# alexkroman/tiny-audio

Measured on AMD Instinct MI355X. Metric: training audio-sec/sec on 10s@16kHz clips, higher is better.
Workload: dtype bf16

## Files before the change

### tiny_audio_amd/csrc/attention.hip

```cpp
#include <cstdlib>
#include <type_traits>
#include "common.h"
#include "../../include/ta355.h"

#define KV_TILE 64
#define CT_STRIDE 128
#define LOG2E 1.4426950408889634f
#define NEG_BIG (-1.0e30f)

#ifdef TA355_ATTN_STAMPS
__device__ unsigned long long g_attn_stamps[8192 * 16];
#define ATTN_STAMP(blk, i, who) do { if (threadIdx.x == (who)) g_attn_stamps[(long)(blk) * 16 + (i)] = __builtin_amdgcn_s_memtime(); } while (0)
extern "C" int ta_debug_attn_stamps(unsigned long long* host_out, int nblocks) {
  return hipMemcpyFromSymbol(host_out, HIP_SYMBOL(g_attn_stamps), (size_t)nblocks * 16 * sizeof(unsigned long long)) == hipSuccess ? 0 : 2;
}
#else
#define ATTN_STAMP(blk, i, who) do { } while (0)
#endif

template <int HD> struct RowTile {
  static constexpr int STRIDE = HD * 2;
  static constexpr int BYTES = 64 * STRIDE;
  static __device__ __forceinline__ int swz(int r) { return HD == 64 ? ((r >> 1) & 7) : (r & 15); }
  static __device__ __forceinline__ int off(int r, int c) { return r * STRIDE + ((c ^ swz(r)) << 4); }
// ... 372 lines not shown
#pragma unroll
          for (int r = 0; r < 4; ++r) {
            const int key = key0 + kt * 16 + g * 4 + r;
            const bool v = (key <= qrow) & (mkv[r] != 0);
            s[sub][kt][r] = v ? s[sub][kt][r] : -INFINITY;
          }
        }
      }
      float mloc = max3(s[sub][0][0], s[sub][0][1], s[sub][0][2]);
      mloc = max3(mloc, s[sub][0][3], s[sub][1][0]);
      mloc = max3(mloc, s[sub][1][1], s[sub][1][2]);
      mloc = max3(mloc, s[sub][1][3], s[sub][2][0]);
      mloc = max3(mloc, s[sub][2][1], s[sub][2][2]);
      mloc = max3(mloc, s[sub][2][3], s[sub][3][0]);
      mloc = max3(mloc, s[sub][3][1], s[sub][3][2]);
      mloc = fmaxf(mloc, s[sub][3][3]);
      const float m_new = fmaxf(m_run[sub], group_max(mloc));
      if (__any(m_new != m_run[sub])) {
        const float alpha = __builtin_amdgcn_exp2f((m_run[sub] - m_new) * sl2);
#pragma unroll
        for (int i = 0; i <= ND; ++i) { o[sub][i][0] *= alpha; o[sub][i][1] *= alpha; o[sub][i][2] *= alpha; o[sub][i][3] *= alpha; }
        m_run[sub] = m_new;
      }
      const float mb = m_new * sl2;
#pragma unroll
      for (int kt = 0; kt < 4; ++kt)
#pragma unroll
        for (int r = 0; r < 4; ++r) s[sub][kt][r] = __builtin_amdgcn_exp2f(fmaf(s[sub][kt][r], sl2, -mb));
    }
#pragma unroll
    for (int kp = 0; kp < 2; ++kp) {
      bf16x8 pb[QSUB];
#pragma unroll
      for (int sub = 0; sub < QSUB; ++sub) pb[sub] = pack_p(s[sub][2 * kp], s[sub][2 * kp + 1]);
#pragma unroll
      for (int dt = 0; dt <= ND; ++dt) {
        const bf16x8 va = read_colfrag(Vt, dt * 16 + l15, (2 * kp) * 16 + g * 4, (2 * kp + 1) * 16 + g * 4);
#pragma unroll
        for (int sub = 0; sub < QSUB; ++sub)
          o[sub][dt] = __builtin_amdgcn_mfma_f32_16x16x32_bf16(va, pb[sub], o[sub][dt], 0, 0, 0);
        if (dt & 1) __builtin_amdgcn_sched_barrier(0);
      }
    }
  }
#pragma unroll
  for (int sub = 0; sub < QSUB; ++sub) {
    const int qrow = q0 + sub * 16 + l15;
    const float l_run = __shfl(o[sub][ND][0], l15, 64);
    if (qrow < L) {
      const float inv = l_run > 0.f ? 1.0f / l_run : 0.f;
      bf16_t* orow = O + ((long)b * L + qrow) * ((long)Hq * HD) + (long)h * HD;
#pragma unroll
      for (int dt = 0; dt < ND; dt += 2) {
        const uint32_t x0 = pack2bf(o[sub][dt][0] * inv, o[sub][dt][1] * inv), x1 = pack2bf(o[sub][dt][2] * inv, o[sub][dt][3] * inv);
        const uint32_t y0 = pack2bf(o[sub][dt + 1][0] * inv, o[sub][dt + 1][1] * inv), y1 = pack2bf(o[sub][dt + 1][2] * inv, o[sub][dt + 1][3] * inv);
        const auto a = __builtin_amdgcn_permlane16_swap(x0, y0, false, false);
        const auto c = __builtin_amdgcn_permlane16_swap(x1, y1, false, false);
        *(uint4*)(orow + 16 * (dt + (g & 1)) + 8 * (g >> 1)) = make_uint4(a[0], c[0], a[1], c[1]);
      }
      if (LSE && g == 0) LSE[(long)(b * Hq + h) * L + qrow] = l_run > 0.f ? m_run[sub] * scale + __logf(l_run) : 1.0e30f;
    }
  }
  }
}

__device__ __forceinline__ void dma16_asm(const void* g, unsigned lds) {
  asm volatile("s_mov_b32 m0, %0\n\ts_nop 0\n\tglobal_load_lds_dwordx4 %1, off" ::"s"(lds), "v"(g) : "memory");
}
__device__ __forceinline__ void dma_rowtile128(const bf16_t* base, long row_stride, int row0, int nrows, unsigned lds_tile, int wave,
                                               int lane) {
#pragma unroll
  for (int i = 0; i < 4; ++i) {
    const int blk = wave + 4 * i, r = blk * 4 + (lane >> 4);
    int gr = row0 + r; if (gr > nrows - 1) gr = nrows - 1; if (gr < 0) gr = 0;
    const int c = (lane & 15) ^ RowTile<128>::swz_tr(r);
    dma16_asm(base + (long)gr * row_stride + c * 8, __builtin_amdgcn_readfirstlane(lds_tile + blk * 1024));
  }
}
__device__ __forceinline__ unsigned lds_addr_of(const char* p) {
  return __builtin_amdgcn_readfirstlane((unsigned)(unsigned long)(const __attribute__((address_space(3))) char*)p);
}
constexpr int BWD_BUF = 2 * 64 * 128 * 2 + 512;

template <int HD, int MAXT, int QSUB, int NW, bool PAIR = false, bool NORM = true, bool ROPE = true>
__global__ __launch_bounds__(NW * 64) void attn_fwd_gqa_qkv_kernel(const bf16_t* __restrict__ qkv0, const float* __restrict__ qn_w,
                                                               const float* __restrict__ kn_w, const float* __restrict__ cosT,
                                                               const float* __restrict__ sinT, const int* __restrict__ pos,
                                                               bf16_t* __restrict__ Qo, bf16_t* __restrict__ Ko, bf16_t* __restrict__ Vo,
                                                               float* __restrict__ rq, float* __restrict__ rk, bf16_t* __restrict__ O,
                                                               float* __restrict__ LSE, const int* __restrict__ kmask, int B, int Hq,
                                                               int Hkv, int L, float scale, float eps) {
  static_assert(HD == 128, "Qwen3 head_dim");
  extern __shared__ __attribute__((aligned(16))) char smem[];
  constexpr int ND = HD / 16, NT_ = NW * 64;
  char* Ks = smem;
  char* Vs = smem + MAXT * RowTile<HD>::BYTES;
  int* Ms = (int*)(Vs + MAXT * RowTile<HD>::BYTES);
  const int tid = threadIdx.x, lane = tid & 63, wave = tid >> 6, g = lane >> 4, l15 = lane & 15;
  const int b = blockIdx.x / Hkv, hk = blockIdx.x % Hkv;
  const int grp = Hq / Hkv, cph = PAIR ? (L + 15) / 16 : (L + 16 * QSUB - 1) / (16 * QSUB), nchunk = PAIR ? cph : grp * cph;
  const long ld = (long)(Hq + 2 * Hkv) * HD;
  const float sl2 = scale * LOG2E;
  const int ntiles = (L + KV_TILE - 1) / KV_TILE;
  constexpr int PER = (MAXT * 64 * (HD / 8) + NT_ - 1) / NT_;
  ATTN_STAMP(blockIdx.x + 6144, 0, 0);
  {
    const unsigned ldsK = lds_addr_of(Ks), ldsV = lds_addr_of(Vs);
    const bf16_t* kbase = qkv0 + (long)b * L * ld + (long)(Hq + hk) * HD;
    const bf16_t* vbase = kbase + (long)Hkv * HD;
    for (int blk = wave; blk < ntiles * 16; blk += NW) {
      const int t = blk >> 4, rb4 = (blk & 15) * 4, r = rb4 + (lane >> 4);
      int gr = t * KV_TILE + r; if (gr > L - 1) gr = L - 1;
      const int c = (lane & 15) ^ RowTile<HD>::swz(r), cv = (lane & 15) ^ RowTile<HD>::swz_tr(r);
      const unsigned off = __builtin_amdgcn_readfirstlane((unsigned)(t * RowTile<HD>::BYTES + rb4 * 256));
      dma16_asm(kbase + (long)gr * ld + c * 8, ldsK + off);
      dma16_asm(vbase + (long)gr * ld + cv * 8, ldsV + off);
    }
  }
  {
    const int c = tid & 15;
    float wk[8];
    if constexpr (NORM) {
      const float4 wa = *(const float4*)(kn_w + c * 8), wb = *(const float4*)(kn_w + c * 8 + 4);
      wk[0] = wa.x; wk[1] = wa.y; wk[2] = wa.z; wk[3] = wa.w; wk[4] = wb.x; wk[5] = wb.y; wk[6] = wb.z; wk[7] = wb.w;
    }
    float4 cc[2][4];
    auto rope_rows = [&](int i, float4* dst) {
      if constexpr (!ROPE) return;
      const int ch = tid + i * NT_, t = ch / (64 * (HD / 8)), w = ch % (64 * (HD / 8));
      const int krow = t * KV_TILE + w / (HD / 8), gr = krow > L - 1 ? L - 1 : krow;
      const int pp = pos ? pos[(long)b * L + gr] : gr;
      const float* cp = cosT + (long)pp * 64 + (c & 7) * 8;
      const float* sp = sinT + (long)pp * 64 + (c & 7) * 8;
      dst[0] = *(const float4*)cp; dst[1] = *(const float4*)(cp + 4); dst[2] = *(const float4*)sp; dst[3] = *(const float4*)(sp + 4);
    };
    rope_rows(0, cc[0]);
    for (int i = tid; i < ntiles * 64; i += NT_) Ms[i] = (i < L) ? (kmask ? kmask[(long)b * L + i] : 1) : 0;
    ATTN_STAMP(blockIdx.x + 6144, 1, 0);
    asm volatile("s_waitcnt vmcnt(0)" ::: "memory");
    __syncthreads();
    ATTN_STAMP(blockIdx.x + 6144, 2, 0);
#pragma unroll
    for (int i = 0; i < PER; ++i) {
      const int ch = tid + i * NT_, t = ch / (64 * (HD / 8)), w = ch % (64 * (HD / 8));
      if (i + 1 < PER) rope_rows(i + 1, cc[(i + 1) & 1]);
      if (t < ntiles) {
        const int r = w / (HD / 8);
        const int krow = t * KV_TILE + r, gr = krow > L - 1 ? L - 1 : krow;
        const long tok = (long)b * L + gr;
        char* kp = Ks + t * RowTile<HD>::BYTES + RowTile<HD>::off(r, c);
        const uint4 kin = *(const uint4*)kp;
        const uint4 vin = *(const uint4*)(Vs + t * RowTile<HD>::BYTES + RowTile<HD>::off_tr(r, c));
        const uint32_t u[4] = {kin.x, kin.y, kin.z, kin.w};
        uint4 kv = kin;
        float rr = 1.f;
        if constexpr (NORM || ROPE) {
          float x[8];
#pragma unroll
          for (int k = 0; k < 4; ++k) { x[2 * k] = bf2f((bf16_t)(u[k] & 0xffff)); x[2 * k + 1] = bf2f((bf16_t)(u[k] >> 16)); }
          if constexpr (NORM) {
            float ss = 0.f;
#pragma unroll
            for (int e = 0; e < 8; ++e) ss += x[e] * x[e];
            ss = row_sum16(ss);
            rr = rsqrtf(ss / (float)HD + eps);
          }
          const float4* q4 = cc[i & 1];
          float cs[8], sn[8];
          if constexpr (ROPE) {
            cs[0] = q4[0].x; cs[1] = q4[0].y; cs[2] = q4[0].z; cs[3] = q4[0].w; cs[4] = q4[1].x; cs[5] = q4[1].y; cs[6] = q4[1].z; cs[7] = q4[1].w;
            sn[0] = q4[2].x; sn[1] = q4[2].y; sn[2] = q4[2].z; sn[3] = q4[2].w; sn[4] = q4[3].x; sn[5] = q4[3].y; sn[6] = q4[3].z; sn[7] = q4[3].w;
          }
          float y[8];
#pragma unroll
          for (int e = 0; e < 8; ++e) {
            const float n = NORM ? x[e] * rr * wk[e] : x[e];
            if constexpr (ROPE) {
              const float np = row_xor8(n);
              y[e] = c < 8 ? n * cs[e] - np * sn[e] : n * cs[e] + np * sn[e];
            } else {
              y[e] = n;
            }
          }
          kv = make_uint4(pack2bf(y[0], y[1]), pack2bf(y[2], y[3]), pack2bf(y[4], y[5]), pack2bf(y[6], y[7]));
          *(uint4*)kp = kv;
        }
        if (krow < L) {
          *(uint4*)(Ko + ((long)(b * Hkv + hk) * L + krow) * HD + c * 8) = kv;
          if (Vo) *(uint4*)(Vo + ((long)(b * Hkv + hk) * L + krow) * HD + c * 8) = vin;
          if (NORM && c == 0) rk[tok * Hkv + hk] = rr;
        }
      }
    }
  }
  ATTN_STAMP(blockIdx.x + 6144, 3, 0);
  __syncthreads();
  ATTN_STAMP(blockIdx.x + 6144, 4, 0);
  const bf16x8 ones = (bf16x8){0x3f80, 0x3f80, 0x3f80, 0x3f80, 0x3f80, 0x3f80, 0x3f80, 0x3f80};
  const bf16x8 zeros = (bf16x8){0, 0, 0, 0, 0, 0, 0, 0};
  const bf16x8 one_row = l15 == 0 ? ones : zeros;
  for (int pass = 0; pass < 2; ++pass) {
  const int chunk = pass == 0 ? wave : nchunk - 1 - wave;
  if (chunk >= nchunk || (pass == 1 && chunk < NW)) continue;
  const int h0 = PAIR ? hk * grp : hk * grp + chunk / cph;
  const int q0 = PAIR ? chunk * 16 : (chunk % cph) * 16 * QSUB;
  constexpr int RSTEP = PAIR ? 0 : 16;
  bf16x8 qf[QSUB][HD / 32];
  float4 tc[2][2], ts[2][2];
#pragma unroll
  for (int sub = 0; sub < QSUB; ++sub) {
    const int h = PAIR ? h0 + sub : h0;
    const int qrow = q0 + sub * RSTEP + l15, qr = qrow > L - 1 ? L - 1 : qrow;
    const long tok = (long)b * L + qr;
    const bf16_t* src = qkv0 + tok * ld + (long)h * HD;
    uint4 raw[HD / 32];
#pragma unroll
    for (int ks = 0; ks < HD / 32; ++ks) raw[ks] = *(const uint4*)(src + ks * 32 + g * 8);
    if (ROPE && (!PAIR || sub == 0)) {
      const int p = pos ? pos[tok] : qr;
#pragma unroll
      for (int ks = 0; ks < 2; ++ks) {
        const int d0 = ks * 32 + g * 8;
        tc[ks][0] = *(const float4*)(cosT + (long)p * 64 + d0); tc[ks][1] = *(const float4*)(cosT + (long)p * 64 + d0 + 4);
        ts[ks][0] = *(const float4*)(sinT + (long)p * 64 + d0); ts[ks][1] = *(const float4*)(sinT + (long)p * 64 + d0 + 4);
      }
    }
    float x[HD / 32][8], ss = 0.f;
#pragma unroll
    for (int ks = 0; ks < HD / 32; ++ks) {
      const uint32_t u[4] = {raw[ks].x, raw[ks].y, raw[ks].z, raw[ks].w};
#pragma unroll
      for (int k = 0; k < 4; ++k) { x[ks][2 * k] = bf2f((bf16_t)(u[k] & 0xffff)); x[ks][2 * k + 1] = bf2f((bf16_t)(u[k] >> 16)); }
      if constexpr (NORM) {
#pragma unroll
        for (int e = 0; e < 8; ++e) ss += x[ks][e] * x[ks][e];
      }
    }
    float rr = 1.f;
    if constexpr (NORM) { ss = group_sum(ss); rr = rsqrtf(ss / (float)HD + eps); }
#pragma unroll
    for (int ks = 0; ks < 2; ++ks) {
      const int d0 = ks * 32 + g * 8;
      float cs[8], sn[8], w1[8], w2[8];
      if constexpr (ROPE) {
        const float4 c0 = tc[ks][0], c1 = tc[ks][1], s0 = ts[ks][0], s1 = ts[ks][1];
        cs[0] = c0.x; cs[1] = c0.y; cs[2] = c0.z; cs[3] = c0.w; cs[4] = c1.x; cs[5] = c1.y; cs[6] = c1.z; cs[7] = c1.w;
        sn[0] = s0.x; sn[1] = s0.y; sn[2] = s0.z; sn[3] = s0.w; sn[4] = s1.x; sn[5] = s1.y; sn[6] = s1.z; sn[7] = s1.w;
      }
      if constexpr (NORM) {
        const float4 wa = *(const float4*)(qn_w + d0), wb = *(const float4*)(qn_w + d0 + 4);
        const float4 wc = *(const float4*)(qn_w + 64 + d0), wd = *(const float4*)(qn_w + 64 + d0 + 4);
        w1[0] = wa.x; w1[1] = wa.y; w1[2] = wa.z; w1[3] = wa.w; w1[4] = wb.x; w1[5] = wb.y; w1[6] = wb.z; w1[7] = wb.w;
        w2[0] = wc.x; w2[1] = wc.y; w2[2] = wc.z; w2[3] = wc.w; w2[4] = wd.x; w2[5] = wd.y; w2[6] = wd.z; w2[7] = wd.w;
      }
      float y1[8], y2[8];
#pragma unroll
      for (int e = 0; e < 8; ++e) {
        const float n1 = NORM ? x[ks][e] * rr * w1[e] : x[ks][e], n2 = NORM ? x[ks + 2][e] * rr * w2[e] : x[ks + 2][e];
        y1[e] = ROPE ? n1 * cs[e] - n2 * sn[e] : n1;
        y2[e] = ROPE ? n2 * cs[e] + n1 * sn[e] : n2;
      }
      union { bf16x8 v; uint4 u; } a, c;
      a.u = make_uint4(pack2bf(y1[0], y1[1]), pack2bf(y1[2], y1[3]), pack2bf(y1[4], y1[5]), pack2bf(y1[6], y1[7]));
      c.u = make_uint4(pack2bf(y2[0], y2[1]), pack2bf(y2[2], y2[3]), pack2bf(y2[4], y2[5]), pack2bf(y2[6], y2[7]));
      qf[sub][ks] = a.v; qf[sub][ks + 2] = c.v;
      if (qrow < L) {
        bf16_t* qdst = Qo + ((long)(b * Hq + h) * L + qrow) * HD;
        *(uint4*)(qdst + d0) = a.u;
        *(uint4*)(qdst + 64 + d0) = c.u;
      }
    }
    if (NORM && qrow < L && g == 0) rq[tok * Hq + h] = rr;
  }
  f32x4 o[QSUB][ND + 1];
#pragma unroll
  for (int sub = 0; sub < QSUB; ++sub)
#pragma unroll
    for (int i = 0; i <= ND; ++i) o[sub][i] = (f32x4){0.f, 0.f, 0.f, 0.f};
  float m_run[QSUB];
#pragma unroll
  for (int sub = 0; sub < QSUB; ++sub) m_run[sub] = NEG_BIG;
  const int my_tiles = min(ntiles, (q0 + (PAIR ? 16 : 16 * QSUB) - 1) / KV_TILE + 1);
  ATTN_STAMP(blockIdx.x + 6144, 5 + 3 * pass, 0);
  for (int t = 0; t < my_tiles; ++t) {
    const int key0 = t * KV_TILE;
    const char* Kt = Ks + t * RowTile<HD>::BYTES;
    const char* Vt = Vs + t * RowTile<HD>::BYTES;
    f32x4 s[QSUB][4];
#pragma unroll
    for (int kt = 0; kt < 4; ++kt) {
#pragma unroll
      for (int sub = 0; sub < QSUB; ++sub) s[sub][kt] = (f32x4){0.f, 0.f, 0.f, 0.f};
#pragma unroll
      for (int ks = 0; ks < HD / 32; ++ks) {
        const bf16x8 a = *(const bf16x8*)(Kt + RowTile<HD>::off(kt * 16 + l15, ks * 4 + g));
#pragma unroll
        for (int sub = 0; sub < QSUB; ++sub)
          s[sub][kt] = __builtin_amdgcn_mfma_f32_16x16x32_bf16(a, qf[sub][ks], s[sub][kt], 0, 0, 0);
      }
      __builtin_amdgcn_sched_barrier(0);
    }
#pragma unroll
    for (int sub = 0; sub < QSUB; ++sub) {
      const int qrow = q0 + sub * RSTEP + l15;
      const bool full = (key0 + KV_TILE <= L) && (kmask == nullptr) && (key0 + KV_TILE - 1 <= q0 + sub * RSTEP);
      if (!full) {
#pragma unroll
        for (int kt = 0; kt < 4; ++kt) {
          const int4 mk = *(const int4*)(Ms + key0 + kt * 16 + g * 4);
          const int mkv[4] = {mk.x, mk.y, mk.z, mk.w};
#pragma unroll
          for (int r = 0; r < 4; ++r) {
            const int key = key0 + kt * 16 + g * 4 + r;
            const bool v = (key <= qrow) & (mkv[r] != 0);
            s[sub][kt][r] = v ? s[sub][kt][r] : -INFINITY;
          }
        }
      }
      float mloc = max3(s[sub][0][0], s[sub][0][1], s[sub][0][2]);
      mloc = max3(mloc, s[sub][0][3], s[sub][1][0]);
      mloc = max3(mloc, s[sub][1][1], s[sub][1][2]);
      mloc = max3(mloc, s[sub][1][3], s[sub][2][0]);
      mloc = max3(mloc, s[sub][2][1], s[sub][2][2]);
      mloc = max3(mloc, s[sub][2][3], s[sub][3][0]);
      mloc = max3(mloc, s[sub][3][1], s[sub][3][2]);
      mloc = fmaxf(mloc, s[sub][3][3]);
      const float m_new = fmaxf(m_run[sub], group_max(mloc));
      if (__any(m_new != m_run[sub])) {
        const float alpha = __builtin_amdgcn_exp2f((m_run[sub] - m_new) * sl2);
#pragma unroll
        for (int i = 0; i <= ND; ++i) { o[sub][i][0] *= alpha; o[sub][i][1] *= alpha; o[sub][i][2] *= alpha; o[sub][i][3] *= alpha; }
        m_run[sub] = m_new;
      }
      const float mb = m_new * sl2;
#pragma unroll
      for (int kt = 0; kt < 4; ++kt)
#pragma unroll
        for (int r = 0; r < 4; ++r) s[sub][kt][r] = __builtin_amdgcn_exp2f(fmaf(s[sub][kt][r], sl2, -mb));
    }
#pragma unroll
    for (int kp = 0; kp < 2; ++kp) {
      bf16x8 pb[QSUB];
#pragma unroll
      for (int sub = 0; sub < QSUB; ++sub) pb[sub] = pack_p(s[sub][2 * kp], s[sub][2 * kp + 1]);
#pragma unroll
      for (int dt = 0; dt <= ND; ++dt) {
        const bf16x8 va = dt < ND ? read_colfrag_tr<HD>(Vt, dt, l15, (2 * kp) * 16 + g * 4, (2 * kp + 1) * 16 + g * 4) : one_row;
#pragma unroll
        for (int sub = 0; sub < QSUB; ++sub)
          o[sub][dt] = __builtin_amdgcn_mfma_f32_16x16x32_bf16(va, pb[sub], o[sub][dt], 0, 0, 0);
        if (dt & 1) __builtin_amdgcn_sched_barrier(0);
      }
    }
  }
  ATTN_STAMP(blockIdx.x + 6144, 6 + 3 * pass, 0);
#pragma unroll
  for (int sub = 0; sub < QSUB; ++sub) {
    const int h = PAIR ? h0 + sub : h0;
    const int qrow = q0 + sub * RSTEP + l15;
    const float l_run = __shfl(o[sub][ND][0], l15, 64);
    if (qrow < L) {
      const float inv = l_run > 0.f ? 1.0f / l_run : 0.f;
      bf16_t* orow = O + ((long)b * L + qrow) * ((long)Hq * HD) + (long)h * HD;
#pragma unroll
      for (int dt = 0; dt < ND; dt += 2) {
        const uint32_t x0 = pack2bf(o[sub][dt][0] * inv, o[sub][dt][1] * inv), x1 = pack2bf(o[sub][dt][2] * inv, o[sub][dt][3] * inv);
        const uint32_t y0 = pack2bf(o[sub][dt + 1][0] * inv, o[sub][dt + 1][1] * inv), y1 = pack2bf(o[sub][dt + 1][2] * inv, o[sub][dt + 1][3] * inv);
        const auto a = __builtin_amdgcn_permlane16_swap(x0, y0, false, false);
        const auto c = __builtin_amdgcn_permlane16_swap(x1, y1, false, false);
        *(uint4*)(orow + 16 * (dt + (g & 1)) + 8 * (g >> 1)) = make_uint4(a[0], c[0], a[1], c[1]);
      }
      if (LSE && g == 0) LSE[(long)(b * Hq + h) * L + qrow] = l_run > 0.f ? m_run[sub] * scale + __logf(l_run) : 1.0e30f;
    }
  }
  ATTN_STAMP(blockIdx.x + 6144, 7 + 3 * pass, 0);
  }
#ifdef TA355_ATTN_STAMPS
  asm volatile("s_waitcnt vmcnt(0)" ::: "memory");
  ATTN_STAMP(blockIdx.x + 6144, 11, 0);
#endif
}

struct QkvPostBwd {
  const bf16_t* qkv0;
  const float *rq, *rk;
  const float *qn_w, *kn_w;
  const float *cosT, *sinT;
  const int* pos;
  bf16_t* dqkv;
};
constexpr int QP_PITCH = 128 * 4 + 16;
__device__ __forceinline__ float oct_sum8(float v) { return row_sum8(v); }
__device__ __forceinline__ void qkv_stage_f32(char* st, const f32x4* acc, int wave, int l15, int g) {
#pragma unroll
  for (int dt = 0; dt < 8; ++dt)
    *(float4*)(st + (wave * 16 + l15) * QP_PITCH + (dt * 16 + g * 4) * 4) = make_float4(acc[dt][0], acc[dt][1], acc[dt][2], acc[dt][3]);
}
template <bool NORM, bool ROPE>
__device__ __forceinline__ void qkv_post_bwd_tile(const char* st, const QkvPostBwd& F, int sec, int b, int row0, int L, int head,
                                                  int Hq, int Hkv, int tid) {
  constexpr int HD = 128;
  const long ld = (long)(Hq + 2 * Hkv) * HD;
  const int Hs = sec == 0 ? Hq : Hkv, j = tid & 7;
  const long coff = (long)(sec == 0 ? head : (sec == 1 ? Hq + head : Hq + Hkv + head)) * HD;
  float w1[8], w2[8];
  if (NORM && sec < 2) {
    const float* nw = sec == 0 ? F.qn_w : F.kn_w;
    const float4 a = *(const float4*)(nw + 8 * j), b4 = *(const float4*)(nw + 8 * j + 4), c = *(const float4*)(nw + 64 + 8 * j), d = *(const float4*)(nw + 64 + 8 * j + 4);
    w1[0] = a.x; w1[1] = a.y; w1[2] = a.z; w1[3] = a.w; w1[4] = b4.x; w1[5] = b4.y; w1[6] = b4.z; w1[7] = b4.w;
    w2[0] = c.x; w2[1] = c.y; w2[2] = c.z; w2[3] = c.w; w2[4] = d.x; w2[5] = d.y; w2[6] = d.z; w2[7] = d.w;
  }
#pragma unroll
  for (int it = 0; it < 2; ++it) {
    const int tl = (tid >> 3) + it * 32, l = row0 + tl;
    const bool live = l < L;
    const int lc = live ? l : L - 1;
    const long tok = (long)b * L + lc;
    const float* sr = (const float*)(st + tl * QP_PITCH);
    float d1[8], d2[8];
    { const float4 a = *(const float4*)(sr + 8 * j), b4 = *(const float4*)(sr + 8 * j + 4), c = *(const float4*)(sr + 64 + 8 * j), d = *(const float4*)(sr + 64 + 8 * j + 4);
      d1[0] = a.x; d1[1] = a.y; d1[2] = a.z; d1[3] = a.w; d1[4] = b4.x; d1[5] = b4.y; d1[6] = b4.z; d1[7] = b4.w;
      d2[0] = c.x; d2[1] = c.y; d2[2] = c.z; d2[3] = c.w; d2[4] = d.x; d2[5] = d.y; d2[6] = d.z; d2[7] = d.w; }
    if ((NORM || ROPE) && sec < 2) {
      float cs[8], sn[8];
      if constexpr (NORM) {
        const bf16_t* src = F.qkv0 + tok * ld + coff;
        const uint4 xa = *(const uint4*)(src + 8 * j), xb = *(const uint4*)(src + 64 + 8 * j);
        const uint32_t ua[4] = {xa.x, xa.y, xa.z, xa.w}, ub[4] = {xb.x, xb.y, xb.z, xb.w};
        float x1[8], x2[8];
#pragma unroll
        for (int k = 0; k < 4; ++k) {
          x1[2 * k] = bf2f((bf16_t)(ua[k] & 0xffff)); x1[2 * k + 1] = bf2f((bf16_t)(ua[k] >> 16));
          x2[2 * k] = bf2f((bf16_t)(ub[k] & 0xffff)); x2[2 * k + 1] = bf2f((bf16_t)(ub[k] >> 16));
        }
        if constexpr (ROPE) {
          const int p = F.pos ? F.pos[tok] : lc;
          const float4 c0 = *(const float4*)(F.cosT + (long)p * 64 + 8 * j), c1 = *(const float4*)(F.cosT + (long)p * 64 + 8 * j + 4);
          const float4 s0 = *(const float4*)(F.sinT + (long)p * 64 + 8 * j), s1 = *(const float4*)(F.sinT + (long)p * 64 + 8 * j + 4);
          cs[0] = c0.x; cs[1] = c0.y; cs[2] = c0.z; cs[3] = c0.w; cs[4] = c1.x; cs[5] = c1.y; cs[6] = c1.z; cs[7] = c1.w;
          sn[0] = s0.x; sn[1] = s0.y; sn[2] = s0.z; sn[3] = s0.w; sn[4] = s1.x; sn[5] = s1.y; sn[6] = s1.z; sn[7] = s1.w;
        }
        const float r = (sec == 0 ? F.rq : F.rk)[tok * Hs + head];
        float dot = 0.f;
#pragma unroll
        for (int e = 0; e < 8; ++e) {
          const float dn1 = ROPE ? d1[e] * cs[e] + d2[e] * sn[e] : d1[e], dn2 = ROPE ? d2[e] * cs[e] - d1[e] * sn[e] : d2[e];
          x1[e] *= r; x2[e] *= r;
          d1[e] = dn1 * w1[e]; d2[e] = dn2 * w2[e];
          dot += d1[e] * x1[e] + d2[e] * x2[e];
        }
        const float md = oct_sum8(dot) / (float)HD;
#pragma unroll
        for (int e = 0; e < 8; ++e) { d1[e] = r * (d1[e] - x1[e] * md); d2[e] = r * (d2[e] - x2[e] * md); }
// ... 305 lines not shown
                                   const ta_attn_layout* lay_in, hipStream_t st) {
  if (B <= 0 || L <= 0) return TA_OK;
  if (Hq % Hkv || Lp % 64 || Lp < L) return TA_ERR_ARG;
  if (!lay_in) {
    const int grp = Hq / Hkv;
    if (head_dim == 128 && causal && L <= 192 && grp * ((L + 31) / 32) <= 12) {
      constexpr int MAXT = 3, QS = 2, NW = 6;
      const size_t lds = MAXT * (RowTile<128>::BYTES + (128 + 16) * CT_STRIDE) + MAXT * 64 * 4;
      static bool attr = false;
      if (!attr) { (void)hipFuncSetAttribute((const void*)attn_fwd_gqa_kernel<128, MAXT, QS, NW>, hipFuncAttributeMaxDynamicSharedMemorySize, (int)lds); attr = true; }
      TA_LAUNCH((attn_fwd_gqa_kernel<128, MAXT, QS, NW>), dim3(B * Hkv), dim3(NW * 64), lds, st, (const bf16_t*)Q, (const bf16_t*)K,
                (const bf16_t*)VT, (bf16_t*)O, LSE, kmask, B, Hq, Hkv, L, Lp, scale);
      TA_CHECK_LAUNCH();
      return TA_OK;
    }
  }
  const long hd = head_dim;
  ta_attn_layout lay = {Hq * L * hd, L * hd, hd, Hkv * L * hd, L * hd, hd, Hkv * hd * Lp, hd * Lp, Lp};
  if (lay_in) lay = *lay_in;
  if (((lay.q_bs | lay.q_hs | lay.q_rs | lay.k_bs | lay.k_hs | lay.k_rs) & 7) || (((uintptr_t)Q | (uintptr_t)K) & 15)) return TA_ERR_ARG;
  const long vor = lay.v_bs | lay.v_hs | lay.v_rs;
  const uintptr_t vp = (uintptr_t)VT;
  int valign = (!(vor & 7) && !(vp & 15)) ? 0 : ((!(vor & 3) && !(vp & 7)) ? 1 : 2);
  const int qsub = (head_dim == 64) ? 2 : 1;
  dim3 grid(grouped_grid((Hq / Hkv) * ta_cdiv(L, 64 * qsub), B * Hkv)), blk(256);
#define FWD(HD_, C_)                                                                                              \
  TA_LAUNCH((attn_fwd_kernel<HD_, C_, (HD_ == 64 ? 2 : 1)>), grid, blk, fwd_lds<HD_>(), st, (const bf16_t*)Q, (const bf16_t*)K, \
                     (const bf16_t*)VT, (bf16_t*)O, LSE, kmask, B, Hq, Hkv, L, Lp, scale, lay, valign)
  if (head_dim == 64 && !causal) FWD(64, false);
  else if (head_dim == 64 && causal) FWD(64, true);
  else if (head_dim == 128 && causal) FWD(128, true);
  else if (head_dim == 128 && !causal) FWD(128, false);
  else return TA_ERR_ARG;
  TA_CHECK_LAUNCH();
  return TA_OK;
}

static int attention_bwd_launch(const void* Q, const void* K, const void* V, const void* dO, long dO_stride, const float* LSE,
                                const float* Delta, const int* kmask, void* dQ, void* dK, void* dV, int B, int Hq, int Hkv, int L,
                                int Lp, int head_dim, int causal, float scale, const QkvPostBwd& F, hipStream_t st) {
  if (!Delta) return TA_ERR_ARG;
  if (B <= 0 || L <= 0) return TA_OK;
  if (Hq % Hkv || Lp % 64 || Lp < L || head_dim != 128) return TA_ERR_ARG;
  constexpr int HD = 128;
  const size_t lds_kv = (2 * (size_t)BWD_BUF > 64 * (size_t)QP_PITCH) ? 2 * (size_t)BWD_BUF : 64 * (size_t)QP_PITCH;
  const bool norm = !F.qkv0 || F.qn_w, rope = !F.qkv0 || F.cosT;
  if (!causal && !(norm && rope)) return TA_ERR_ARG;
  static bool attr_done = false;
  if (!attr_done) {
    (void)hipFuncSetAttribute((const void*)attn_bwd_kernel<HD, true>, hipFuncAttributeMaxDynamicSharedMemorySize, (int)lds_kv);
    (void)hipFuncSetAttribute((const void*)attn_bwd_kernel<HD, false>, hipFuncAttributeMaxDynamicSharedMemorySize, (int)lds_kv);
    (void)hipFuncSetAttribute((const void*)attn_bwd_kernel<HD, true, true, false>, hipFuncAttributeMaxDynamicSharedMemorySize, (int)lds_kv);
    (void)hipFuncSetAttribute((const void*)attn_bwd_kernel<HD, true, false, true>, hipFuncAttributeMaxDynamicSharedMemorySize, (int)lds_kv);
    (void)hipFuncSetAttribute((const void*)attn_bwd_kernel<HD, true, false, false>, hipFuncAttributeMaxDynamicSharedMemorySize, (int)lds_kv);
    attr_done = true;
  }
  const int n_dq = grouped_grid((Hq / Hkv) * ta_cdiv(L, 64), B * Hkv), n_dkv = grouped_grid(ta_cdiv(L, 64), B * Hkv);
  dim3 grid(n_dq + n_dkv), blk(256);
  const bf16_t* nul = nullptr;
#define BWD(...)                                                                                                                    \
  TA_LAUNCH((attn_bwd_kernel<HD, __VA_ARGS__>), grid, blk, lds_kv, st, (const bf16_t*)Q, nul, (const bf16_t*)K, nul, (const bf16_t*)V, \
            (const bf16_t*)dO, dO_stride, nul, LSE, Delta, kmask, (bf16_t*)dQ, (bf16_t*)dK, (bf16_t*)dV, B, Hq, Hkv, L, Lp, scale, n_dkv, F)
  if (!causal) BWD(false);
  else if (norm && rope) BWD(true);
  else if (norm) BWD(true, true, false);
  else if (rope) BWD(true, false, true);
  else BWD(true, false, false);
#undef BWD
  TA_CHECK_LAUNCH();
  return TA_OK;
}

extern "C" int ta_attention_fwd_qkv(const void* qkv0, const float* qn_w, const float* kn_w, const float* cosT, const float* sinT,
                                    const int* pos, void* Q, void* K, void* V, float* rq, float* rk, void* O, float* LSE,
                                    const int* kmask, int B, int Hq, int Hkv, int L, float scale, float eps, hipStream_t st) {
  if (B <= 0 || L <= 0) return TA_OK;
  if (!qkv0 || !Q || !K || !O || Hkv <= 0 || Hq % Hkv) return TA_ERR_ARG;
  if (!qn_w != !kn_w || !cosT != !sinT) return TA_ERR_ARG;
  const bool norm = qn_w != nullptr, rope = cosT != nullptr;
  if (norm && (!rq || !rk)) return TA_ERR_ARG;
  const int grp = Hq / Hkv;
  if (L > 192 || grp * ((L + 31) / 32) > 12) return TA_ERR_ARG;
  constexpr int MAXT = 3, QS = 2, NW = 6;
  const size_t lds = 2 * MAXT * RowTile<128>::BYTES + MAXT * 64 * 4;
  static bool attr = false;
#define FQ_ATTR(...) (void)hipFuncSetAttribute((const void*)attn_fwd_gqa_qkv_kernel<128, MAXT, QS, NW, __VA_ARGS__>, hipFuncAttributeMaxDynamicSharedMemorySize, (int)lds)
  if (!attr) {
    FQ_ATTR(false); FQ_ATTR(true);
    FQ_ATTR(false, true, false); FQ_ATTR(true, true, false); FQ_ATTR(false, false, true); FQ_ATTR(true, false, true);
    FQ_ATTR(false, false, false); FQ_ATTR(true, false, false);
    attr = true;
  }
#undef FQ_ATTR
#define FQ(...)                                                                                                                       \
  TA_LAUNCH((attn_fwd_gqa_qkv_kernel<128, MAXT, QS, NW, __VA_ARGS__>), dim3(B * Hkv), dim3(NW * 64), lds, st, (const bf16_t*)qkv0, qn_w, kn_w, \
            cosT, sinT, pos, (bf16_t*)Q, (bf16_t*)K, (bf16_t*)V, rq, rk, (bf16_t*)O, LSE, kmask, B, Hq, Hkv, L, scale, eps)
  const bool pair = grp == 2;
  if (norm && rope) { if (pair) FQ(true); else FQ(false); }
  else if (norm) { if (pair) FQ(true, true, false); else FQ(false, true, false); }
  else if (rope) { if (pair) FQ(true, false, true); else FQ(false, false, true); }
  else { if (pair) FQ(true, false, false); else FQ(false, false, false); }
#undef FQ
  TA_CHECK_LAUNCH();
  return TA_OK;
}

extern "C" int ta_attention_bwd(const void* Q, const void* QT, const void* K, const void* KT, const void* V,
                                const void* dO, long dO_stride, const void* dOT, const float* LSE, const float* Delta,
                                const int* kmask, void* dQ, void* dK, void* dV, int B, int Hq, int Hkv, int L, int Lp,
                                int head_dim, int causal, float scale, hipStream_t st) {
  (void)QT; (void)KT; (void)dOT;
  QkvPostBwd F = {};
  return attention_bwd_launch(Q, K, V, dO, dO_stride, LSE, Delta, kmask, dQ, dK, dV, B, Hq, Hkv, L, Lp, head_dim, causal, scale, F, st);
}

extern "C" int ta_attention_bwd_qkv(const void* Q, const void* K, const void* V, const void* dO, long dO_stride, const float* LSE,
                                    const float* Delta, const int* kmask, const void* qkv0, const float* rq, const float* rk,
                                    const float* qn_w, const float* kn_w, const float* cosT, const float* sinT, const int* pos,
                                    void* dqkv, int B, int Hq, int Hkv, int L, int Lp, int head_dim, int causal, float scale,
                                    hipStream_t st) {
  if (!qkv0 || !dqkv || !qn_w != !kn_w || !cosT != !sinT || (qn_w && (!rq || !rk))) return TA_ERR_ARG;
  QkvPostBwd F = {(const bf16_t*)qkv0, rq, rk, qn_w, kn_w, cosT, sinT, pos, (bf16_t*)dqkv};
  return attention_bwd_launch(Q, K, V, dO, dO_stride, LSE, Delta, kmask, nullptr, nullptr, nullptr, B, Hq, Hkv, L, Lp, head_dim, causal,
                              scale, F, st);
}
```

Before: 7731.

## Prefetch query rows and RoPE tables alongside K/V DMA in fused attention forward

```diff
diff --git a/tiny_audio_amd/csrc/attention.hip b/tiny_audio_amd/csrc/attention.hip
--- a/tiny_audio_amd/csrc/attention.hip
+++ b/tiny_audio_amd/csrc/attention.hip
@@ -478,6 +478,7 @@
 }
 constexpr int BWD_BUF = 2 * 64 * 128 * 2 + 512;
 
+#define TA_WAIT_VMCNT(n) do { asm volatile("" ::: "memory"); __builtin_amdgcn_s_waitcnt(0x0F70 | (n)); asm volatile("" ::: "memory"); } while (0)
 template <int HD, int MAXT, int QSUB, int NW, bool PAIR = false, bool NORM = true, bool ROPE = true>
 __global__ __launch_bounds__(NW * 64) void attn_fwd_gqa_qkv_kernel(const bf16_t* __restrict__ qkv0, const float* __restrict__ qn_w,
                                                                const float* __restrict__ kn_w, const float* __restrict__ cosT,
@@ -489,184 +490,265 @@
   static_assert(HD == 128, "Qwen3 head_dim");
   extern __shared__ __attribute__((aligned(16))) char smem[];
   constexpr int ND = HD / 16, NT_ = NW * 64;
+  constexpr int NTB = PAIR ? 1 : QSUB;
+  static_assert(MAXT * 64 <= NT_, "one key-mask entry per thread");
+  constexpr int NVW = MAXT * 16 / NW;
+  static_assert(MAXT * 16 % NW == 0 && NVW < 16, "every wave issues the same number of V DMA instructions");
   char* Ks = smem;
   char* Vs = smem + MAXT * RowTile<HD>::BYTES;
   int* Ms = (int*)(Vs + MAXT * RowTile<HD>::BYTES);
   const int tid = threadIdx.x, lane = tid & 63, wave = tid >> 6, g = lane >> 4, l15 = lane & 15;
+  float* RkS = (float*)(Ms + MAXT * 64);
+  float* QwS = RkS + MAXT * 64;
+  char* Qs = (char*)(QwS + HD) + wave * (QSUB * (HD / 32) * 1024) + lane * 16;
   const int b = blockIdx.x / Hkv, hk = blockIdx.x % Hkv;
   const int grp = Hq / Hkv, cph = PAIR ? (L + 15) / 16 : (L + 16 * QSUB - 1) / (16 * QSUB), nchunk = PAIR ? cph : grp * cph;
   const long ld = (long)(Hq + 2 * Hkv) * HD;
   const float sl2 = scale * LOG2E;
   const int ntiles = (L + KV_TILE - 1) / KV_TILE;
+  constexpr int RSTEP = PAIR ? 0 : 16;
+  const int chunk0 = wave < nchunk ? wave : -1, chunk1 = nchunk - 1 - wave >= NW ? nchunk - 1 - wave : -1;
+  auto head0 = [&](int chunk) { return PAIR ? hk * grp : hk * grp + chunk / cph; };
+  auto row0 = [&](int chunk) { return PAIR ? chunk * 16 : (chunk % cph) * 16 * QSUB; };
   constexpr int PER = (MAXT * 64 * (HD / 8) + NT_ - 1) / NT_;
+  const int c = tid & 15;
   ATTN_STAMP(blockIdx.x + 6144, 0, 0);
-  {
-    const unsigned ldsK = lds_addr_of(Ks), ldsV = lds_addr_of(Vs);
-    const bf16_t* kbase = qkv0 + (long)b * L * ld + (long)(Hq + hk) * HD;
-    const bf16_t* vbase = kbase + (long)Hkv * HD;
-    for (int blk = wave; blk < ntiles * 16; blk += NW) {
-      const int t = blk >> 4, rb4 = (blk & 15) * 4, r = rb4 + (lane >> 4);
-      int gr = t * KV_TILE + r; if (gr > L - 1) gr = L - 1;
-      const int c = (lane & 15) ^ RowTile<HD>::swz(r), cv = (lane & 15) ^ RowTile<HD>::swz_tr(r);
-      const unsigned off = __builtin_amdgcn_readfirstlane((unsigned)(t * RowTile<HD>::BYTES + rb4 * 256));
-      dma16_asm(kbase + (long)gr * ld + c * 8, ldsK + off);
-      dma16_asm(vbase + (long)gr * ld + cv * 8, ldsV + off);
-    }
-  }
-  {
-    const int c = tid & 15;
-    float wk[8];
-    if constexpr (NORM) {
-      const float4 wa = *(const float4*)(kn_w + c * 8), wb = *(const float4*)(kn_w + c * 8 + 4);
-      wk[0] = wa.x; wk[1] = wa.y; wk[2] = wa.z; wk[3] = wa.w; wk[4] = wb.x; wk[5] = wb.y; wk[6] = wb.z; wk[7] = wb.w;
-    }
-    float4 cc[2][4];
-    auto rope_rows = [&](int i, float4* dst) {
-      if constexpr (!ROPE) return;
-      const int ch = tid + i * NT_, t = ch / (64 * (HD / 8)), w = ch % (64 * (HD / 8));
-      const int krow = t * KV_TILE + w / (HD / 8), gr = krow > L - 1 ? L - 1 : krow;
-      const int pp = pos ? pos[(long)b * L + gr] : gr;
-      const float* cp = cosT + (long)pp * 64 + (c & 7) * 8;
-      const float* sp = sinT + (long)pp * 64 + (c & 7) * 8;
-      dst[0] = *(const float4*)cp; dst[1] = *(const float4*)(cp + 4); dst[2] = *(const float4*)sp; dst[3] = *(const float4*)(sp + 4);
-    };
-    rope_rows(0, cc[0]);
-    for (int i = tid; i < ntiles * 64; i += NT_) Ms[i] = (i < L) ? (kmask ? kmask[(long)b * L + i] : 1) : 0;
-    ATTN_STAMP(blockIdx.x + 6144, 1, 0);
-    asm volatile("s_waitcnt vmcnt(0)" ::: "memory");
-    __syncthreads();
-    ATTN_STAMP(blockIdx.x + 6144, 2, 0);
+  int kpp[PER], qpp[2][NTB];
+#pragma unroll
+  for (int i = 0; i < PER; ++i) {
+    const int krow = (tid + i * NT_) / (HD / 8), gr = krow > L - 1 ? L - 1 : krow;
+    kpp[i] = (ROPE && pos) ? pos[(long)b * L + gr] : gr;
+  }
+#pragma unroll
+  for (int p = 0; p < 2; ++p)
+#pragma unroll
+    for (int s = 0; s < NTB; ++s) {
+      const int chunk = p == 0 ? chunk0 : chunk1;
+      const int qrow = row0(chunk < 0 ? 0 : chunk) + s * RSTEP + l15, qr = qrow > L - 1 ? L - 1 : qrow;
+      qpp[p][s] = (ROPE && pos) ? pos[(long)b * L + qr] : qr;
+    }
+  float4 cc[2][4];
+  auto rope_rows = [&](int pp, float4* dst) {
+    if constexpr (!ROPE) return;
+    const float* cp = cosT + (long)pp * 64 + (c & 7) * 8;
+    const float* sp = sinT + (long)pp * 64 + (c & 7) * 8;
+    dst[0] = *(const float4*)cp; dst[1] = *(const float4*)(cp + 4); dst[2] = *(const float4*)sp; dst[3] = *(const float4*)(sp + 4);
+  };
+  rope_rows(kpp[0], cc[0]);
+  if (PER > 1) rope_rows(kpp[PER > 1 ? 1 : 0], cc[1]);
+  float4 tc[2][NTB][2][2], ts[2][NTB][2][2];
+  uint4 raw[QSUB][HD / 32];
+  auto query_tables = [&](int p) __attribute__((always_inline)) {
+#pragma unroll
+    for (int s = 0; s < NTB; ++s)
+#pragma unroll
+      for (int ks = 0; ks < 2; ++ks) {
+        tc[p][s][ks][0] = tc[p][s][ks][1] = ts[p][s][ks][0] = ts[p][s][ks][1] = make_float4(0.f, 0.f, 0.f, 0.f);
+        if (ROPE && (p == 0 ? chunk0 : chunk1) >= 0) {
+          const int d0 = ks * 32 + g * 8;
+          const float* cp = cosT + (long)qpp[p][s] * 64 + d0;
+          const float* sp = sinT + (long)qpp[p][s] * 64 + d0;
+          tc[p][s][ks][0] = *(const float4*)cp; tc[p][s][ks][1] = *(const float4*)(cp + 4);
+          ts[p][s][ks][0] = *(const float4*)sp; ts[p][s][ks][1] = *(const float4*)(sp + 4);
+        }
+      }
+  };
+  constexpr bool TABLES1_EARLY = PAIR;
+  query_tables(0);
+  if (TABLES1_EARLY) query_tables(1);
+  float wk[8];
+  if constexpr (NORM) {
+    const float4 wa = *(const float4*)(kn_w + c * 8), wb = *(const float4*)(kn_w + c * 8 + 4);
+    wk[0] = wa.x; wk[1] = wa.y; wk[2] = wa.z; wk[3] = wa.w; wk[4] = wb.x; wk[5] = wb.y; wk[6] = wb.z; wk[7] = wb.w;
+  }
+  float4 qwv = make_float4(0.f, 0.f, 0.f, 0.f);
+  if (NORM && tid < HD / 4) qwv = *(const float4*)(qn_w + tid * 4);
+  const int mval = tid < ntiles * 64 ? ((tid < L) ? (kmask ? kmask[(long)b * L + tid] : 1) : 0) : 0;
+  const unsigned ldsK = lds_addr_of(Ks), ldsV = lds_addr_of(Vs);
+  const bf16_t* kbase = qkv0 + (long)b * L * ld + (long)(Hq + hk) * HD;
+  const bf16_t* vbase = kbase + (long)Hkv * HD;
+  for (int blk = wave; blk < ntiles * 16; blk += NW) {
+    const int t = blk >> 4, rb4 = (blk & 15) * 4, r = rb4 + (lane >> 4);
+    int gr = t * KV_TILE + r; if (gr > L - 1) gr = L - 1;
+    const int ck = (lane & 15) ^ RowTile<HD>::swz(r);
+    const unsigned off = __builtin_amdgcn_readfirstlane((unsigned)(t * RowTile<HD>::BYTES + rb4 * 256));
+    dma16_asm(kbase + (long)gr * ld + ck * 8, ldsK + off);
+  }
+#pragma unroll
+  for (int p = 0; p < 2; ++p) {
+    const int chunk = p == 0 ? chunk0 : chunk1;
+    if (p == 0 || chunk >= 0) {
+      const int h0 = head0(chunk < 0 ? 0 : chunk), q0 = row0(chunk < 0 ? 0 : chunk);
+#pragma unroll
+      for (int sub = 0; sub < QSUB; ++sub) {
+        const int h = PAIR ? h0 + sub : h0;
+        const int qrow = q0 + sub * RSTEP + l15, qr = qrow > L - 1 ? L - 1 : qrow;
+        const bf16_t* src = qkv0 + ((long)b * L + qr) * ld + (long)h * HD;
+#pragma unroll
+        for (int ks = 0; ks < HD / 32; ++ks) {
+          if (p == 0) raw[sub][ks] = *(const uint4*)(src + ks * 32 + g * 8);
+          else dma16_asm(src + ks * 32 + g * 8, lds_addr_of(Qs - lane * 16 + (sub * (HD / 32) + ks) * 1024));
+        }
+      }
+    }
+  }
+#pragma unroll
+  for (int j = 0; j < NVW; ++j) {
+    const int blk = wave + j * NW, t = blk >> 4, rb4 = (blk & 15) * 4, r = rb4 + (lane >> 4);
+    int gr = t * KV_TILE + r; if (gr > L - 1) gr = L - 1;
+    const int cv = (lane & 15) ^ RowTile<HD>::swz_tr(r);
+    const unsigned off = __builtin_amdgcn_readfirstlane((unsigned)(t * RowTile<HD>::BYTES + rb4 * 256));
+    dma16_asm(vbase + (long)gr * ld + cv * 8, ldsV + off);
+  }
+  ATTN_STAMP(blockIdx.x + 6144, 1, 0);
+  TA_WAIT_VMCNT(NVW);
+  if (tid < ntiles * 64) Ms[tid] = mval;
+  if (NORM && tid < HD / 4) *(float4*)(QwS + tid * 4) = qwv;
+  __syncthreads();
+  ATTN_STAMP(blockIdx.x + 6144, 2, 0);
+  if constexpr (NORM || ROPE) {
 #pragma unroll
     for (int i = 0; i < PER; ++i) {
       const int ch = tid + i * NT_, t = ch / (64 * (HD / 8)), w = ch % (64 * (HD / 8));
-      if (i + 1 < PER) rope_rows(i + 1, cc[(i + 1) & 1]);
       if (t < ntiles) {
         const int r = w / (HD / 8);
-        const int krow = t * KV_TILE + r, gr = krow > L - 1 ? L - 1 : krow;
-        const long tok = (long)b * L + gr;
         char* kp = Ks + t * RowTile<HD>::BYTES + RowTile<HD>::off(r, c);
         const uint4 kin = *(const uint4*)kp;
-        const uint4 vin = *(const uint4*)(Vs + t * RowTile<HD>::BYTES + RowTile<HD>::off_tr(r, c));
         const uint32_t u[4] = {kin.x, kin.y, kin.z, kin.w};
-        uint4 kv = kin;
         float rr = 1.f;
-        if constexpr (NORM || ROPE) {
-          float x[8];
-#pragma unroll
-          for (int k = 0; k < 4; ++k) { x[2 * k] = bf2f((bf16_t)(u[k] & 0xffff)); x[2 * k + 1] = bf2f((bf16_t)(u[k] >> 16)); }
-          if constexpr (NORM) {
-            float ss = 0.f;
-#pragma unroll
-            for (int e = 0; e < 8; ++e) ss += x[e] * x[e];
-            ss = row_sum16(ss);
-            rr = rsqrtf(ss / (float)HD + eps);
+        float x[8];
+#pragma unroll
+        for (int k = 0; k < 4; ++k) { x[2 * k] = bf2f((bf16_t)(u[k] & 0xffff)); x[2 * k + 1] = bf2f((bf16_t)(u[k] >> 16)); }
+        if constexpr (NORM) {
+          float ss = 0.f;
+#pragma unroll
+          for (int e = 0; e < 8; ++e) ss += x[e] * x[e];
+          ss = row_sum16(ss);
+          rr = rsqrtf(ss / (float)HD + eps);
+        }
+        const float4* q4 = cc[i & 1];
+        float cs[8], sn[8];
+        if constexpr (ROPE) {
+          cs[0] = q4[0].x; cs[1] = q4[0].y; cs[2] = q4[0].z; cs[3] = q4[0].w; cs[4] = q4[1].x; cs[5] = q4[1].y; cs[6] = q4[1].z; cs[7] = q4[1].w;
+          sn[0] = q4[2].x; sn[1] = q4[2].y; sn[2] = q4[2].z; sn[3] = q4[2].w; sn[4] = q4[3].x; sn[5] = q4[3].y; sn[6] = q4[3].z; sn[7] = q4[3].w;
+        }
+        float y[8];
+#pragma unroll
+        for (int e = 0; e < 8; ++e) {
+          const float n = NORM ? x[e] * rr * wk[e] : x[e];
+          if constexpr (ROPE) {
+            const float np = row_xor8(n);
+            y[e] = c < 8 ? n * cs[e] - np * sn[e] : n * cs[e] + np * sn[e];
+          } else {
+            y[e] = n;
           }
-          const float4* q4 = cc[i & 1];
-          float cs[8], sn[8];
-          if constexpr (ROPE) {
-            cs[0] = q4[0].x; cs[1] = q4[0].y; cs[2] = q4[0].z; cs[3] = q4[0].w; cs[4] = q4[1].x; cs[5] = q4[1].y; cs[6] = q4[1].z; cs[7] = q4[1].w;
-            sn[0] = q4[2].x; sn[1] = q4[2].y; sn[2] = q4[2].z; sn[3] = q4[2].w; sn[4] = q4[3].x; sn[5] = q4[3].y; sn[6] = q4[3].z; sn[7] = q4[3].w;
-          }
-          float y[8];
-#pragma unroll
-          for (int e = 0; e < 8; ++e) {
-            const float n = NORM ? x[e] * rr * wk[e] : x[e];
-            if constexpr (ROPE) {
-              const float np = row_xor8(n);
-              y[e] = c < 8 ? n * cs[e] - np * sn[e] : n * cs[e] + np * sn[e];
-            } else {
-              y[e] = n;
-            }
-          }
-          kv = make_uint4(pack2bf(y[0], y[1]), pack2bf(y[2], y[3]), pack2bf(y[4], y[5]), pack2bf(y[6], y[7]));
-          *(uint4*)kp = kv;
-        }
-        if (krow < L) {
-          *(uint4*)(Ko + ((long)(b * Hkv + hk) * L + krow) * HD + c * 8) = kv;
-          if (Vo) *(uint4*)(Vo + ((long)(b * Hkv + hk) * L + krow) * HD + c * 8) = vin;
-          if (NORM && c == 0) rk[tok * Hkv + hk] = rr;
-        }
-      }
+        }
+        *(uint4*)kp = make_uint4(pack2bf(y[0], y[1]), pack2bf(y[2], y[3]), pack2bf(y[4], y[5]), pack2bf(y[6], y[7]));
+        if (NORM && c == 0) RkS[t * KV_TILE + r] = rr;
+      }
+      if (i + 2 < PER) rope_rows(kpp[i + 2 < PER ? i + 2 : 0], cc[i & 1]);
     }
   }
   ATTN_STAMP(blockIdx.x + 6144, 3, 0);
+  if (!TABLES1_EARLY) query_tables(1);
+  TA_WAIT_VMCNT(0);
   __syncthreads();
   ATTN_STAMP(blockIdx.x + 6144, 4, 0);
+#pragma unroll
+  for (int i = 0; i < PER; ++i) {
+    const int ch = tid + i * NT_, t = ch / (64 * (HD / 8)), w = ch % (64 * (HD / 8));
+    const int r = w / (HD / 8), krow = t * KV_TILE + r;
+    if (t < ntiles && krow < L) {
+      const long dst = ((long)(b * Hkv + hk) * L + krow) * HD + c * 8;
+      *(uint4*)(Ko + dst) = *(const uint4*)(Ks + t * RowTile<HD>::BYTES + RowTile<HD>::off(r, c));
+      if (Vo) *(uint4*)(Vo + dst) = *(const uint4*)(Vs + t * RowTile<HD>::BYTES + RowTile<HD>::off_tr(r, c));
+      if (NORM && c == 0) rk[((long)b * L + krow) * Hkv + hk] = RkS[krow];
+    }
+  }
+  bf16x8 qf[QSUB][HD / 32];
+  auto stage_queries = [&](int chunk, const uint4 (&rw)[QSUB][HD / 32], const float4 (&tcp)[NTB][2][2], const float4 (&tsp)[NTB][2][2])
+                           __attribute__((always_inline)) {
+    const int h0 = head0(chunk), q0 = row0(chunk);
+#pragma unroll
+    for (int sub = 0; sub < QSUB; ++sub) {
+      const int h = PAIR ? h0 + sub : h0;
+      const int qrow = q0 + sub * RSTEP + l15, qr = qrow > L - 1 ? L - 1 : qrow;
+      const long tok = (long)b * L + qr;
+      float x[HD / 32][8], ss = 0.f;
+#pragma unroll
+      for (int ks = 0; ks < HD / 32; ++ks) {
+        const uint32_t u[4] = {rw[sub][ks].x, rw[sub][ks].y, rw[sub][ks].z, rw[sub][ks].w};
+#pragma unroll
+        for (int k = 0; k < 4; ++k) { x[ks][2 * k] = bf2f((bf16_t)(u[k] & 0xffff)); x[ks][2 * k + 1] = bf2f((bf16_t)(u[k] >> 16)); }
+        if constexpr (NORM) {
+#pragma unroll
+          for (int e = 0; e < 8; ++e) ss += x[ks][e] * x[ks][e];
+        }
+      }
+      float rr = 1.f;
+      if constexpr (NORM) { ss = group_sum(ss); rr = rsqrtf(ss / (float)HD + eps); }
+#pragma unroll
+      for (int ks = 0; ks < 2; ++ks) {
+        const int d0 = ks * 32 + g * 8;
+        float cs[8], sn[8], w1[8], w2[8];
+        if constexpr (ROPE) {
+          const float4 c0 = tcp[PAIR ? 0 : sub][ks][0], c1 = tcp[PAIR ? 0 : sub][ks][1], s0 = tsp[PAIR ? 0 : sub][ks][0], s1 = tsp[PAIR ? 0 : sub][ks][1];
+          cs[0] = c0.x; cs[1] = c0.y; cs[2] = c0.z; cs[3] = c0.w; cs[4] = c1.x; cs[5] = c1.y; cs[6] = c1.z; cs[7] = c1.w;
+          sn[0] = s0.x; sn[1] = s0.y; sn[2] = s0.z; sn[3] = s0.w; sn[4] = s1.x; sn[5] = s1.y; sn[6] = s1.z; sn[7] = s1.w;
+        }
+        if constexpr (NORM) {
+          const float4 wa = *(const float4*)(QwS + d0), wb = *(const float4*)(QwS + d0 + 4);
+          const float4 wc = *(const float4*)(QwS + 64 + d0), wd = *(const float4*)(QwS + 64 + d0 + 4);
+          w1[0] = wa.x; w1[1] = wa.y; w1[2] = wa.z; w1[3] = wa.w; w1[4] = wb.x; w1[5] = wb.y; w1[6] = wb.z; w1[7] = wb.w;
+          w2[0] = wc.x; w2[1] = wc.y; w2[2] = wc.z; w2[3] = wc.w; w2[4] = wd.x; w2[5] = wd.y; w2[6] = wd.z; w2[7] = wd.w;
+        }
+        float y1[8], y2[8];
+#pragma unroll
+        for (int e = 0; e < 8; ++e) {
+          const float n1 = NORM ? x[ks][e] * rr * w1[e] : x[ks][e], n2 = NORM ? x[ks + 2][e] * rr * w2[e] : x[ks + 2][e];
+          y1[e] = ROPE ? n1 * cs[e] - n2 * sn[e] : n1;
+          y2[e] = ROPE ? n2 * cs[e] + n1 * sn[e] : n2;
+        }
+        union { bf16x8 v; uint4 u; } a, cq;
+        a.u = make_uint4(pack2bf(y1[0], y1[1]), pack2bf(y1[2], y1[3]), pack2bf(y1[4], y1[5]), pack2bf(y1[6], y1[7]));
+        cq.u = make_uint4(pack2bf(y2[0], y2[1]), pack2bf(y2[2], y2[3]), pack2bf(y2[4], y2[5]), pack2bf(y2[6], y2[7]));
+        qf[sub][ks] = a.v; qf[sub][ks + 2] = cq.v;
+        if (qrow < L) {
+          bf16_t* qdst = Qo + ((long)(b * Hq + h) * L + qrow) * HD;
+          *(uint4*)(qdst + d0) = a.u;
+          *(uint4*)(qdst + 64 + d0) = cq.u;
+        }
+      }
+      if (NORM && qrow < L && g == 0) rq[tok * Hq + h] = rr;
+    }
+  };
+  if (chunk1 >= 0) {
+    uint4 raw1[QSUB][HD / 32];
+#pragma unroll
+    for (int sub = 0; sub < QSUB; ++sub)
+#pragma unroll
+      for (int ks = 0; ks < HD / 32; ++ks) raw1[sub][ks] = *(const uint4*)(Qs + (sub * (HD / 32) + ks) * 1024);
+    stage_queries(chunk1, raw1, tc[1], ts[1]);
+#pragma unroll
+    for (int sub = 0; sub < QSUB; ++sub)
+#pragma unroll
+      for (int ks = 0; ks < HD / 32; ++ks) *(bf16x8*)(Qs + (sub * (HD / 32) + ks) * 1024) = qf[sub][ks];
+  }
+  if (chunk0 >= 0) stage_queries(chunk0, raw, tc[0], ts[0]);
   const bf16x8 ones = (bf16x8){0x3f80, 0x3f80, 0x3f80, 0x3f80, 0x3f80, 0x3f80, 0x3f80, 0x3f80};
   const bf16x8 zeros = (bf16x8){0, 0, 0, 0, 0, 0, 0, 0};
   const bf16x8 one_row = l15 == 0 ? ones : zeros;
+  ATTN_STAMP(blockIdx.x + 6144, 5, 0);
   for (int pass = 0; pass < 2; ++pass) {
-  const int chunk = pass == 0 ? wave : nchunk - 1 - wave;
-  if (chunk >= nchunk || (pass == 1 && chunk < NW)) continue;
-  const int h0 = PAIR ? hk * grp : hk * grp + chunk / cph;
-  const int q0 = PAIR ? chunk * 16 : (chunk % cph) * 16 * QSUB;
-  constexpr int RSTEP = PAIR ? 0 : 16;
-  bf16x8 qf[QSUB][HD / 32];
-  float4 tc[2][2], ts[2][2];
-#pragma unroll
-  for (int sub = 0; sub < QSUB; ++sub) {
-    const int h = PAIR ? h0 + sub : h0;
-    const int qrow = q0 + sub * RSTEP + l15, qr = qrow > L - 1 ? L - 1 : qrow;
-    const long tok = (long)b * L + qr;
-    const bf16_t* src = qkv0 + tok * ld + (long)h * HD;
-    uint4 raw[HD / 32];
-#pragma unroll
-    for (int ks = 0; ks < HD / 32; ++ks) raw[ks] = *(const uint4*)(src + ks * 32 + g * 8);
-    if (ROPE && (!PAIR || sub == 0)) {
-      const int p = pos ? pos[tok] : qr;
-#pragma unroll
-      for (int ks = 0; ks < 2; ++ks) {
-        const int d0 = ks * 32 + g * 8;
-        tc[ks][0] = *(const float4*)(cosT + (long)p * 64 + d0); tc[ks][1] = *(const float4*)(cosT + (long)p * 64 + d0 + 4);
-        ts[ks][0] = *(const float4*)(sinT + (long)p * 64 + d0); ts[ks][1] = *(const float4*)(sinT + (long)p * 64 + d0 + 4);
-      }
-    }
-    float x[HD / 32][8], ss = 0.f;
-#pragma unroll
-    for (int ks = 0; ks < HD / 32; ++ks) {
-      const uint32_t u[4] = {raw[ks].x, raw[ks].y, raw[ks].z, raw[ks].w};
-#pragma unroll
-      for (int k = 0; k < 4; ++k) { x[ks][2 * k] = bf2f((bf16_t)(u[k] & 0xffff)); x[ks][2 * k + 1] = bf2f((bf16_t)(u[k] >> 16)); }
-      if constexpr (NORM) {
-#pragma unroll
-        for (int e = 0; e < 8; ++e) ss += x[ks][e] * x[ks][e];
-      }
-    }
-    float rr = 1.f;
-    if constexpr (NORM) { ss = group_sum(ss); rr = rsqrtf(ss / (float)HD + eps); }
-#pragma unroll
-    for (int ks = 0; ks < 2; ++ks) {
-      const int d0 = ks * 32 + g * 8;
-      float cs[8], sn[8], w1[8], w2[8];
-      if constexpr (ROPE) {
-        const float4 c0 = tc[ks][0], c1 = tc[ks][1], s0 = ts[ks][0], s1 = ts[ks][1];
-        cs[0] = c0.x; cs[1] = c0.y; cs[2] = c0.z; cs[3] = c0.w; cs[4] = c1.x; cs[5] = c1.y; cs[6] = c1.z; cs[7] = c1.w;
-        sn[0] = s0.x; sn[1] = s0.y; sn[2] = s0.z; sn[3] = s0.w; sn[4] = s1.x; sn[5] = s1.y; sn[6] = s1.z; sn[7] = s1.w;
-      }
-      if constexpr (NORM) {
-        const float4 wa = *(const float4*)(qn_w + d0), wb = *(const float4*)(qn_w + d0 + 4);
-        const float4 wc = *(const float4*)(qn_w + 64 + d0), wd = *(const float4*)(qn_w + 64 + d0 + 4);
-        w1[0] = wa.x; w1[1] = wa.y; w1[2] = wa.z; w1[3] = wa.w; w1[4] = wb.x; w1[5] = wb.y; w1[6] = wb.z; w1[7] = wb.w;
-        w2[0] = wc.x; w2[1] = wc.y; w2[2] = wc.z; w2[3] = wc.w; w2[4] = wd.x; w2[5] = wd.y; w2[6] = wd.z; w2[7] = wd.w;
-      }
-      float y1[8], y2[8];
-#pragma unroll
-      for (int e = 0; e < 8; ++e) {
-        const float n1 = NORM ? x[ks][e] * rr * w1[e] : x[ks][e], n2 = NORM ? x[ks + 2][e] * rr * w2[e] : x[ks + 2][e];
-        y1[e] = ROPE ? n1 * cs[e] - n2 * sn[e] : n1;
-        y2[e] = ROPE ? n2 * cs[e] + n1 * sn[e] : n2;
-      }
-      union { bf16x8 v; uint4 u; } a, c;
-      a.u = make_uint4(pack2bf(y1[0], y1[1]), pack2bf(y1[2], y1[3]), pack2bf(y1[4], y1[5]), pack2bf(y1[6], y1[7]));
-      c.u = make_uint4(pack2bf(y2[0], y2[1]), pack2bf(y2[2], y2[3]), pack2bf(y2[4], y2[5]), pack2bf(y2[6], y2[7]));
-      qf[sub][ks] = a.v; qf[sub][ks + 2] = c.v;
-      if (qrow < L) {
-        bf16_t* qdst = Qo + ((long)(b * Hq + h) * L + qrow) * HD;
-        *(uint4*)(qdst + d0) = a.u;
-        *(uint4*)(qdst + 64 + d0) = c.u;
-      }
-    }
-    if (NORM && qrow < L && g == 0) rq[tok * Hq + h] = rr;
+  const int chunk = pass == 0 ? chunk0 : chunk1;
+  if (chunk < 0) continue;
+  const int h0 = head0(chunk), q0 = row0(chunk);
+  if (pass == 1) {
+#pragma unroll
+    for (int sub = 0; sub < QSUB; ++sub)
+#pragma unroll
+      for (int ks = 0; ks < HD / 32; ++ks) qf[sub][ks] = *(const bf16x8*)(Qs + (sub * (HD / 32) + ks) * 1024);
+    ATTN_STAMP(blockIdx.x + 6144, 8, 0);
   }
   f32x4 o[QSUB][ND + 1];
 #pragma unroll
@@ -677,7 +759,6 @@
 #pragma unroll
   for (int sub = 0; sub < QSUB; ++sub) m_run[sub] = NEG_BIG;
   const int my_tiles = min(ntiles, (q0 + (PAIR ? 16 : 16 * QSUB) - 1) / KV_TILE + 1);
-  ATTN_STAMP(blockIdx.x + 6144, 5 + 3 * pass, 0);
   for (int t = 0; t < my_tiles; ++t) {
     const int key0 = t * KV_TILE;
     const char* Kt = Ks + t * RowTile<HD>::BYTES;
@@ -763,8 +844,8 @@
         const uint32_t x0 = pack2bf(o[sub][dt][0] * inv, o[sub][dt][1] * inv), x1 = pack2bf(o[sub][dt][2] * inv, o[sub][dt][3] * inv);
         const uint32_t y0 = pack2bf(o[sub][dt + 1][0] * inv, o[sub][dt + 1][1] * inv), y1 = pack2bf(o[sub][dt + 1][2] * inv, o[sub][dt + 1][3] * inv);
         const auto a = __builtin_amdgcn_permlane16_swap(x0, y0, false, false);
-        const auto c = __builtin_amdgcn_permlane16_swap(x1, y1, false, false);
-        *(uint4*)(orow + 16 * (dt + (g & 1)) + 8 * (g >> 1)) = make_uint4(a[0], c[0], a[1], c[1]);
+        const auto cq = __builtin_amdgcn_permlane16_swap(x1, y1, false, false);
+        *(uint4*)(orow + 16 * (dt + (g & 1)) + 8 * (g >> 1)) = make_uint4(a[0], cq[0], a[1], cq[1]);
       }
       if (LSE && g == 0) LSE[(long)(b * Hq + h) * L + qrow] = l_run > 0.f ? m_run[sub] * scale + __logf(l_run) : 1.0e30f;
     }
@@ -1236,7 +1317,7 @@
   const int grp = Hq / Hkv;
   if (L > 192 || grp * ((L + 31) / 32) > 12) return TA_ERR_ARG;
   constexpr int MAXT = 3, QS = 2, NW = 6;
-  const size_t lds = 2 * MAXT * RowTile<128>::BYTES + MAXT * 64 * 4;
+  const size_t lds = 2 * MAXT * RowTile<128>::BYTES + 2 * MAXT * 64 * 4 + 128 * 4 + NW * QS * 4 * 1024;
   static bool attr = false;
 #define FQ_ATTR(...) (void)hipFuncSetAttribute((const void*)attn_fwd_gqa_qkv_kernel<128, MAXT, QS, NW, __VA_ARGS__>, hipFuncAttributeMaxDynamicSharedMemorySize, (int)lds)
   if (!attr) {
```

After: 7756 (median of 6 runs). No clear change (+0.3%).
